# tzt101/MichiGAN

Hardware: AMD Instinct MI355X
Metric: training images/sec at 512x512 (G+D step) (higher is better)
Workload: dtype bf16; 1 GPU; SPADEB G + multiscale PatchGAN D + VGG19 + Gabor orientation losses, full G step + D step (Adam), bs=8/GPU, 512x512, BASELINE.json configs[2]; global_batch=8, batch_per_gpu=8, resolution=512, parallelism=dp1, init=reference default (xavier, 0.02), random VGG weights

## Files before the change

### michigan_amd/csrc/mg_conv_halo64.hip

```cpp
#include "mg_conv_common.h"

namespace {

constexpr int H64_PW = 18;
constexpr int H64_ROWS = H64_PW * H64_PW;
constexpr int H64_PINSTR = 44;
constexpr int H64_THREADS = 512;
constexpr int H64_PIPW = (H64_PINSTR + 7) / 8;
constexpr int H64_PBUF = H64_PINSTR * 1024;
constexpr int H64_PAR = 2 * H64_PBUF;
constexpr int H64_AUX = H64_PAR + 256;
constexpr int H64_LTMAX = 4;
constexpr int H64_LDS = H64_AUX + 8 * 4096 + H64_LTMAX * 8192;
constexpr int H64_W8 = H64_AUX + 8 * 4096;
template <int AUX> struct H64Taps { static constexpr int RT = 6, LT = 9 - RT; };
constexpr int H64_NST = 8;

struct Halo64Args {
    int units;
    int mtiles;
    int nseg;
    int tiles_per_seg;
    int bands;
    int dbg;
};

template <int ACT, int AUX>
__global__ __launch_bounds__(H64_THREADS, 2) void conv3x3_halo64_kernel(const ConvK d, const Halo64Args g)
{
    extern __shared__ __attribute__((aligned(16))) unsigned char smem[];
    const int tid = threadIdx.x, lane = tid & 63;
    const int wave = __builtin_amdgcn_readfirstlane(tid >> 6);
    const int pw = wave & 3, mw = wave >> 2;
    const int l31 = lane & 31, hi = lane >> 5;
    constexpr int H64_RT = H64Taps<AUX>::RT, H64_LT = H64Taps<AUX>::LT;

    int unit = blockIdx.x;
    if ((g.units & 7) == 0) unit = (blockIdx.x & 7) * (g.units >> 3) + (blockIdx.x >> 3);
    const int m = unit % g.mtiles;  unit /= g.mtiles;
    const int seg = unit % g.nseg;  unit /= g.nseg;
    const int band = unit % g.bands;
    const int img = unit / g.bands;
    const int m0 = m * 64 + mw * 32, y0 = band * 16, xs = seg * g.tiles_per_seg * 16;
    const int W = d.Win, H = d.Hin;

    const uint16_t* __restrict__ In = reinterpret_cast<const uint16_t*>(d.in);
    const unsigned lds0 = (unsigned)(size_t)(__attribute__((address_space(3))) unsigned char*)smem;

    bf16x8_t a[2][H64_RT][2];
    {
        const uint16_t* __restrict__ Wt = reinterpret_cast<const uint16_t*>(d.wt);
#pragma unroll
        for (int t = 0; t < H64_RT; ++t) {
            const uint16_t* row = Wt + ((size_t)t * d.CoutP + m0 + l31) * 64 + hi * 8;
#pragma unroll
            for (int c = 0; c < 2; ++c)
#pragma unroll
                for (int ks = 0; ks < 2; ++ks)
                    a[c][t][ks] = *reinterpret_cast<const bf16x8_t*>(row + c * 32 + ks * 16);
        }
    }
#pragma unroll
    for (int lt = 0; lt < H64_LT; ++lt) {
        const int row = wave * 8 + (lane >> 3), piece = (lane & 7) ^ ((row >> 1) & 7);
        glds16(reinterpret_cast<const uint16_t*>(d.wt) + ((size_t)(H64_RT + lt) * d.CoutP + m * 64 + row) * 64 + piece * 8,
               __builtin_amdgcn_readfirstlane(lds0 + H64_W8 + lt * 8192 + wave * 1024));
    }
    const int a8off = H64_W8 + (mw * 32 + l31) * 128 + ((hi ^ ((l31 >> 1) & 7)) << 4);
    if (wave == 0) {
        const void* src = (d.bias && m * 64 + lane < d.Cout_gemm) ? static_cast<const void*>(d.bias + m * 64 + lane) : static_cast<const void*>(g_mg_zeros + lane * 4);
        glds4(src, __builtin_amdgcn_readfirstlane(lds0 + H64_PAR));
    }
    const float* const par = reinterpret_cast<const float*>(smem + H64_PAR) + mw * 32;

    const unsigned char* const zsrc = g_mg_zeros + (lane & 7) * 16;
    int poff[H64_PIPW];
#pragma unroll
    for (int j = 0; j < H64_PIPW; ++j) {
        const int q = (wave + 8 * j) * 8 + (lane >> 3), s = lane & 7;
        const int pr = q / H64_PW, pc = q - pr * H64_PW;
        const int iy = y0 + pr - 1, ix = xs + pc - 1;
        const int piece = s ^ ((q >> 1) & 7);
        const bool rowok = q < H64_ROWS && (unsigned)iy < (unsigned)H;
        poff[j] = rowok ? ((int)((((long)(img * H + iy) * W + ix) * 64 + piece * 8) * 2) | (pc == 0 ? 1 : (pc == H64_PW - 1 ? 2 : 0))) : 3;
    }
    auto issue_patch = [&](int i) {
        const unsigned base = lds0 + (i & 1) * H64_PBUF;
        const int x0 = xs + i * 16;
        const bool lok = x0 > 0, rok = x0 + 16 < W;
#pragma unroll
        for (int j = 0; j < H64_PIPW; ++j) {
            if (wave + 8 * j >= H64_PINSTR) continue;
            const int cls = poff[j] & 3;
            const bool ok = cls == 0 || (cls == 1 && lok) || (cls == 2 && rok);
            const unsigned char* src = ok ? reinterpret_cast<const unsigned char*>(In) + ((long)(poff[j] & ~3) + (long)i * (16 * 64 * 2)) : zsrc;
            glds16(src, __builtin_amdgcn_readfirstlane(base + (wave + 8 * j) * 1024));
        }
    };

    int bbase[9][2];
    {
        const int py = l31 >> 4, px = (l31 - 2 * py) & 15;
#pragma unroll
        for (int t = 0; t < 9; ++t) {
            const int tp = d.tap[t];
            const int dy = (int)(short)(tp & 0xffff), dx = tp >> 16;
#pragma unroll
            for (int nt = 0; nt < 2; ++nt) {
                const int q = (pw * 4 + nt * 2 + py + 1 + dy) * H64_PW + px + 1 + dx;
                bbase[t][nt] = q * 128 + ((hi ^ ((q >> 1) & 7)) << 4);
            }
        }
    }
    unsigned ooff[2];
#pragma unroll
    for (int nt = 0; nt < 2; ++nt) {
        const int p = pw * 64 + nt * 32 + l31, py = p >> 4;
        const int y = y0 + py, x = xs + (((p & 15) - 2 * (py & 1)) & 15);
        ooff[nt] = (unsigned)(((img * d.Hout + y) * d.Wout + x) * d.Cout + m0);
    }
    uint16_t* __restrict__ Out = reinterpret_cast<uint16_t*>(d.out);
    const uint16_t* __restrict__ Aux = reinterpret_cast<const uint16_t*>(AUX == 1 ? d.resid : d.x);
    const float neg = ACT == 2 ? d.slope : 0.f;

    issue_patch(0);
    wait_vmcnt<0>();

    for (int i = 0; i < g.tiles_per_seg; ++i) {
        __builtin_amdgcn_s_barrier();
        if (i + 1 < g.tiles_per_seg && !(g.dbg & 2)) issue_patch(i + 1);
        if constexpr (AUX != 0) {
            const unsigned abase = lds0 + H64_AUX + wave * 4096;
            const uint16_t* const asrc = Aux + (hi ? ooff[1] : ooff[0]);
#pragma unroll
            for (int gq = 0; gq < 4; ++gq) glds16(asrc + gq * 8, __builtin_amdgcn_readfirstlane(abase + gq * 1024));
        }
        f32x16_t acc[2];
        const unsigned char* const Ps = smem + (i & 1) * H64_PBUF;
        if (g.dbg & 4) {
#pragma unroll
            for (int nt = 0; nt < 2; ++nt)
#pragma unroll
                for (int r = 0; r < 16; ++r) acc[nt][r] = 0.f;
        } else {
#pragma unroll
        for (int c = 0; c < 2; ++c)
#pragma unroll
            for (int t = 0; t < 9; ++t)
#pragma unroll
                for (int ks = 0; ks < 2; ++ks) {
                    bf16x8_t b[2], at;
#pragma unroll
                    for (int nt = 0; nt < 2; ++nt)
                        b[nt] = *reinterpret_cast<const bf16x8_t*>(Ps + (bbase[t][nt] ^ ((c * 4 + ks * 2) << 4)));
                    if (t < H64_RT) at = a[c][t < H64_RT ? t : 0][ks];
                    else at = *reinterpret_cast<const bf16x8_t*>(smem + (t - H64_RT) * 8192 + (a8off ^ ((c * 4 + ks * 2) << 4)));
#pragma unroll
                    for (int nt = 0; nt < 2; ++nt) {
                        if (c == 0 && t == 0 && ks == 0) {
                            const f32x16_t zero = {};
                            acc[nt] = __builtin_amdgcn_mfma_f32_32x32x16_bf16(at, b[nt], zero, 0, 0, 0);
                        } else
                            acc[nt] = __builtin_amdgcn_mfma_f32_32x32x16_bf16(at, b[nt], acc[nt], 0, 0, 0);
                    }
                }
        }
        wait_vmcnt<0>();

#pragma unroll
        for (int nt = 0; nt < 2; ++nt)
#pragma unroll
            for (int k2 = 0; k2 < 2; ++k2) {
                mg_pk2 v[4];
#pragma unroll
                for (int r2 = 0; r2 < 2; ++r2) {
                    const int rq = 2 * k2 + r2;
                    const f32x4_t bias4 = *reinterpret_cast<const f32x4_t*>(par + hi * 4 + rq * 8);
                    f32x4_t ax = {};
                    if constexpr (AUX != 0) {
                        const uint2 r = *reinterpret_cast<const uint2*>(smem + H64_AUX + wave * 4096 + rq * 1024 + (nt * 32 + l31) * 16 + hi * 8);
                        ax[0] = __uint_as_float(r.x << 16); ax[1] = __uint_as_float(r.x & 0xffff0000u);
                        ax[2] = __uint_as_float(r.y << 16); ax[3] = __uint_as_float(r.y & 0xffff0000u);
                    }
#pragma unroll
                    for (int h2 = 0; h2 < 2; ++h2) {
                        mg_pk2 tt = mg_pk(acc[nt][rq * 4 + 2 * h2], acc[nt][rq * 4 + 2 * h2 + 1]) + mg_pk(bias4[2 * h2], bias4[2 * h2 + 1]);
                        if constexpr (AUX == 1) tt += mg_pk(ax[2 * h2], ax[2 * h2 + 1]);
                        tt = mg_act2<ACT>(tt, neg);
                        if constexpr (AUX == 2) {
                            const mg_pk2 tm = tt * d.mslope;
                            tt[0] = ax[2 * h2] > 0.f ? tt[0] : tm[0];
                            tt[1] = ax[2 * h2 + 1] > 0.f ? tt[1] : tm[1];
                        }
                        v[r2 * 2 + h2] = tt;
                    }
                }
                const uint4 w = mg_pair_swap(mg_pack_bf16x2x2(v[0], v[1]), mg_pack_bf16x2x2(v[2], v[3]));
                if (!(g.dbg & 1)) *reinterpret_cast<uint4*>(Out + ooff[nt] + k2 * 16 + hi * 8) = w;
                else if (w.x == 0x12345678u) *reinterpret_cast<uint4*>(Out) = w;
            }
#pragma unroll
        for (int nt = 0; nt < 2; ++nt) ooff[nt] += 16 * d.Cout;
    }
}

template <int ACT, int AUX>
int launch64(const ConvK& k, const Halo64Args& g, hipStream_t st)
{
    auto kern = conv3x3_halo64_kernel<ACT, AUX>;
    mg_raise_lds_cap(reinterpret_cast<const void*>(kern), H64_LDS);
    hipLaunchKernelGGL(kern, dim3((unsigned)g.units), dim3(H64_THREADS), H64_LDS, st, k, g);
    MG_CHECK_LAUNCH("mg_conv_taps(halo64)");
    return MG_OK;
}

int aux_kind(const ConvK& k) { return k.resid ? (k.x ? 3 : 1) : (k.x ? 2 : 0); }
int act_kind(const ConvK& k) { return (k.act == MG_ACT_LRELU && !(k.slope >= 0.f && k.slope <= 1.f)) ? 3 : k.act; }

}

bool conv_halo64_applies(const ConvK& k, int dtype, int epilogue)
{
    if (!mg_opt(MG_OPT_CONV_HALO) || !mg_opt(MG_OPT_CONV_HALO64) || dtype != MG_BF16 || epilogue != MG_EPI_PLAIN) return false;
    if (k.Cin != 64 || k.Cout != k.Cout_gemm || (k.Cout % 64) != 0 || k.CoutP < k.Cout) return false;
    if (k.ntaps != 9 || k.isy != 1 || k.isx != 1 || k.osy != 1 || k.osx != 1 || k.ooy != 0 || k.oox != 0) return false;
    if (k.Hj != k.Hin || k.Wj != k.Win || k.Hout != k.Hin || k.Wout != k.Win) return false;
    if ((k.Hin % 16) || (k.Win % 16) || k.Hin < 32 || k.Win < 32) return false;
    if (!(k.wide & 1) || (k.wide & ~1)) return false;
    const int ak = aux_kind(k), ck = act_kind(k);
    if (!((ak == 0 && ck <= 2) || (ak <= 2 && ck == 0))) return false;
    if ((long)k.N * k.Hin * k.Win * 64 * 2 >= (1L << 31) || (long)k.N * k.Hin * k.Win * k.Cout >= (1L << 32)) return false;
    unsigned seen = 0;
    for (int t = 0; t < 9; ++t) {
        const int dy = (int)(short)(k.tap[t] & 0xffff), dx = k.tap[t] >> 16;
        if (dy < -1 || dy > 1 || dx < -1 || dx > 1) return false;
        seen |= 1u << ((dy + 1) * 3 + dx + 1);
    }
    if (seen != 0x1ffu) return false;
    if (k.Cout > 128) return false;
    return (long)k.N * (k.Hin / 16) * (k.Win / 16) * (k.Cout / 64) >= 1024;
}

int launch_conv_halo64(ConvK& k, hipStream_t st)
{
    Halo64Args g;
    g.mtiles = k.Cout / 64;
    g.bands = k.Hin / 16;
    const int tiles_x = k.Win / 16;
    const long strips = (long)k.N * g.bands * g.mtiles;
    int nseg = 1;
    while (strips * nseg < 256 && (tiles_x % (nseg * 2)) == 0 && tiles_x / (nseg * 2) >= 4) nseg *= 2;
    g.nseg = nseg;
    g.tiles_per_seg = tiles_x / nseg;
    g.units = (int)(strips * nseg);
    g.dbg = mg_opt(MG_OPT_PROBE_HALO64_DBG);
    const int ak = aux_kind(k), ck = act_kind(k);
    if (ak == 1) return launch64<0, 1>(k, g, st);
    if (ak == 2) return launch64<0, 2>(k, g, st);
    if (ck == 0) return launch64<0, 0>(k, g, st);
    if (ck == 1) return launch64<1, 0>(k, g, st);
    return launch64<2, 0>(k, g, st);
}
```

### michigan_amd/csrc/mg_conv_thin.hip

```cpp
#include "mg_conv_common.h"
#include "mg_launch.h"
#include "mg_wgrad_common.h"


namespace {

constexpr int THIN_TH = 8, THIN_TW = 32;
constexpr int THIN_HW = THIN_TW + 2, THIN_HH = THIN_TH + 2;
constexpr int THIN_HALO_BYTES = THIN_HH * THIN_HW * 16;

template <int CS>
__global__ __launch_bounds__(256, 4) void conv3x3_thin_kernel(const ConvK d, const int ntiles)
{
    constexpr int NB = 2;
    constexpr int CH = NB * 4;
    constexpr int ROW = NB * 64;
    constexpr int RPW = 2 * CS;
    extern __shared__ __attribute__((aligned(16))) unsigned char smem[];
    unsigned char* const halo = smem;
    float* const bias_s = reinterpret_cast<float*>(smem + THIN_HALO_BYTES);
    const int tid = threadIdx.x, lane = tid & 63, wave = tid >> 6, l31 = lane & 31, hi = lane >> 5;
    const int half = CS == 2 ? (wave >> 1) : 0, r0 = CS == 2 ? (wave & 1) * RPW : wave * RPW;
    const int cb = half * 64;
    unsigned char* const stage = smem + THIN_HALO_BYTES + CS * 64 * 4 + wave * (32 * ROW);

    if (tid < CS * 64) bias_s[tid] = (d.bias && tid < d.Cout_gemm) ? d.bias[tid] : 0.f;

    bf16x8_t wa[5][NB];
    int boff[5];
    const uint16_t* __restrict__ Wt = reinterpret_cast<const uint16_t*>(d.wt);
#pragma unroll
    for (int s = 0; s < 5; ++s) {
        const int t = 2 * s + hi;
        const int tc = t < 9 ? t : 8;
        const int dy = (int)(short)(d.tap[tc] & 0xffff), dx = d.tap[tc] >> 16;
        boff[s] = ((1 + dy) * THIN_HW + (1 + dx) + l31) * 16;
#pragma unroll
        for (int nb = 0; nb < NB; ++nb) {
            bf16x8_t z = {0, 0, 0, 0, 0, 0, 0, 0};
            if (t < 9) z = *reinterpret_cast<const bf16x8_t*>(Wt + ((size_t)t * d.CoutP + cb + nb * 32 + l31) * 8);
            wa[s][nb] = z;
        }
    }

    const float neg = mg_neg_slope(d.act, d.slope);
    const bool relu = d.act == MG_ACT_RELU;
    const uint16_t* __restrict__ In = reinterpret_cast<const uint16_t*>(d.in);
    unsigned char* __restrict__ Out = reinterpret_cast<unsigned char*>(d.out);
    const int tpi = d.tiles_y * d.tiles_x;

    for (int tile = blockIdx.x; tile < ntiles; tile += gridDim.x) {
        const int img = tile / tpi, tr = tile - img * tpi;
        const int y0 = (tr / d.tiles_x) * THIN_TH, x0 = (tr % d.tiles_x) * THIN_TW;
        __syncthreads();
#pragma unroll
        for (int it = 0; it < 2; ++it) {
            const int i = tid + it * 256;
            if (i < THIN_HH * THIN_HW) {
                const int hy = i / THIN_HW, hx = i - hy * THIN_HW;
                const int gy = y0 - 1 + hy, gx = x0 - 1 + hx;
                uint4 v = {0u, 0u, 0u, 0u};
                if (gy >= 0 && gy < d.Hin && gx >= 0 && gx < d.Win)
                    v = *reinterpret_cast<const uint4*>(In + ((size_t)(img * d.Hin + gy) * d.Win + gx) * 8);
                *reinterpret_cast<uint4*>(halo + i * 16) = v;
            }
        }
        __syncthreads();
#pragma unroll 1
        for (int mb = 0; mb < RPW; ++mb) {
            const int r = r0 + mb, y = y0 + r;
            if (y >= d.Hin) break;
            bf16x8_t b[5];
#pragma unroll
            for (int s = 0; s < 5; ++s) b[s] = *reinterpret_cast<const bf16x8_t*>(halo + boff[s] + r * (THIN_HW * 16));
            f32x16_t acc[NB];
#pragma unroll
            for (int nb = 0; nb < NB; ++nb)
#pragma unroll
                for (int g = 0; g < 4; ++g) {
                    const f32x4_t bq = *reinterpret_cast<const f32x4_t*>(bias_s + cb + nb * 32 + g * 8 + hi * 4);
#pragma unroll
                    for (int e = 0; e < 4; ++e) acc[nb][g * 4 + e] = bq[e];
                }
#pragma unroll
            for (int s = 0; s < 5; ++s)
#pragma unroll
                for (int nb = 0; nb < NB; ++nb)
                    acc[nb] = __builtin_amdgcn_mfma_f32_32x32x16_bf16(wa[s][nb], b[s], acc[nb], 0, 0, 0);
#pragma unroll
            for (int nb = 0; nb < NB; ++nb)
#pragma unroll
                for (int g = 0; g < 4; ++g) {
                    uint2 u;
                    u.x = f2bf2(mg_act_fast(acc[nb][g * 4 + 0], neg, relu), mg_act_fast(acc[nb][g * 4 + 1], neg, relu));
                    u.y = f2bf2(mg_act_fast(acc[nb][g * 4 + 2], neg, relu), mg_act_fast(acc[nb][g * 4 + 3], neg, relu));
                    const int c = nb * 4 + g;
                    *reinterpret_cast<uint2*>(stage + l31 * ROW + ((c ^ ((l31 >> 1) & (CH - 1))) << 4) + hi * 8) = u;
                }
            __builtin_amdgcn_fence(__ATOMIC_RELEASE, "wavefront");
            __builtin_amdgcn_wave_barrier();
            const size_t orow = (size_t)(img * d.Hout + y) * d.Wout + x0;
#pragma unroll
            for (int it = 0; it < CH / 2; ++it) {
                const int q = it * 64 + lane;
                const int p = q / CH, c = q % CH;
                const uint4 v = *reinterpret_cast<const uint4*>(stage + p * ROW + ((c ^ ((p >> 1) & (CH - 1))) << 4));
                const int co = cb + c * 8;
                if (co < d.Cout)
                    *reinterpret_cast<uint4*>(Out + ((orow + p) * d.Cout + co) * 2) = v;
            }
            __builtin_amdgcn_fence(__ATOMIC_ACQUIRE, "wavefront");
            __builtin_amdgcn_wave_barrier();
        }
    }
}

template <int CS>
int launch_thin(ConvK& k, hipStream_t st)
{
    k.tiles_y = (k.Hin + THIN_TH - 1) / THIN_TH;
    k.tiles_x = k.Win / THIN_TW;
    const long ntiles = (long)k.N * k.tiles_y * k.tiles_x;
    if (ntiles <= 0 || ntiles > 0x7fffffffL) return mg_fail(MG_ERR_ARG, "mg_conv_taps(thin): bad grid %ld", ntiles);
    const int lds = THIN_HALO_BYTES + CS * 64 * 4 + 4 * 32 * 128;
    const long grid = ntiles < 1024 ? ntiles : 1024;
    hipLaunchKernelGGL(conv3x3_thin_kernel<CS>, dim3((unsigned)grid), dim3(256), lds, st, k, (int)ntiles);
    MG_CHECK_LAUNCH("mg_conv_taps(thin)");
    return MG_OK;
}


template <int CS, int S>
__global__ __launch_bounds__(256, 2) void conv_thin_taps_kernel(const ConvK d, const int ntiles, const int HH, const int HW,
                                                                const int dy0, const int dx0, const int nsteps)
{
    constexpr int NB = 2, CH = NB * 4, ROW = NB * 64, RPW = 2 * CS, RB = 2, WROWS = CS * 64;
    extern __shared__ __attribute__((aligned(16))) unsigned char smem[];
    const int tid = threadIdx.x, lane = tid & 63, wave = tid >> 6, l31 = lane & 31, hi = lane >> 5;
    const int half = CS == 2 ? (wave >> 1) : 0, r0 = CS == 2 ? (wave & 1) * RPW : wave * RPW;
    const int cb = half * 64;
    unsigned char* const wl = smem;
    unsigned char* const halo = wl + nsteps * 2 * WROWS * 16;
    int* const tofs = reinterpret_cast<int*>(halo + HH * HW * 16);
    float* const bias_s = reinterpret_cast<float*>(tofs + MG_MAX_TAPS);
    unsigned char* const stage = reinterpret_cast<unsigned char*>(bias_s + WROWS) + wave * (32 * ROW);

    if (tid < WROWS) bias_s[tid] = (d.bias && tid < d.Cout_gemm) ? d.bias[tid] : 0.f;
    if (tid < MG_MAX_TAPS) {
        int v = 0;
#pragma unroll
        for (int t = 0; t < MG_MAX_TAPS; ++t) v = (tid == t) ? d.tap[t] : v;
        tofs[tid] = v;
    }
    {
        const uint16_t* __restrict__ Wt = reinterpret_cast<const uint16_t*>(d.wt);
        for (int i = tid; i < nsteps * 2 * WROWS; i += 256) {
            const int t = i / WROWS, row = i % WROWS;
            uint4 v = {0u, 0u, 0u, 0u};
            if (t < d.ntaps) v = *reinterpret_cast<const uint4*>(Wt + ((size_t)t * d.CoutP + row) * 8);
            *reinterpret_cast<uint4*>(wl + i * 16) = v;
        }
    }
    const float neg = mg_neg_slope(d.act, d.slope);
    const bool relu = d.act == MG_ACT_RELU;
    const uint16_t* __restrict__ In = reinterpret_cast<const uint16_t*>(d.in);
    unsigned char* __restrict__ Out = reinterpret_cast<unsigned char*>(d.out);
    const int tpi = d.tiles_y * d.tiles_x;
    const unsigned char* const wa = wl + (hi * WROWS + cb + l31) * 16;

    constexpr int HPT = 6;
    uint4 hv[HPT];
    const int npix = HH * HW;
    auto fetch = [&](int tile) {
        const int img = tile / tpi, tr = tile - img * tpi;
        const int y0 = (tr / d.tiles_x) * THIN_TH, x0 = (tr % d.tiles_x) * THIN_TW;
#pragma unroll
        for (int q = 0; q < HPT; ++q) {
            const int i = tid + q * 256;
            const int hy = i / HW, hx = i - hy * HW;
            const int gy = y0 * S + dy0 + hy, gx = x0 * S + dx0 + hx;
            uint4 v = {0u, 0u, 0u, 0u};
            if (i < npix && gy >= 0 && gy < d.Hin && gx >= 0 && gx < d.Win)
                v = *reinterpret_cast<const uint4*>(In + ((size_t)(img * d.Hin + gy) * d.Win + gx) * 8);
            hv[q] = v;
        }
    };
    if ((int)blockIdx.x < ntiles) fetch(blockIdx.x);
    for (int tile = blockIdx.x; tile < ntiles; tile += gridDim.x) {
        const int img = tile / tpi, tr = tile - img * tpi;
        const int y0 = (tr / d.tiles_x) * THIN_TH, x0 = (tr % d.tiles_x) * THIN_TW;
        __syncthreads();
#pragma unroll
        for (int q = 0; q < HPT; ++q) {
            const int i = tid + q * 256;
            if (i < npix) *reinterpret_cast<uint4*>(halo + i * 16) = hv[q];
        }
        __syncthreads();
        if (tile + (int)gridDim.x < ntiles) fetch(tile + gridDim.x);
#pragma unroll 1
        for (int rg = 0; rg < RPW; rg += RB) {
        if (y0 + r0 + rg >= d.Hj) break;
        const unsigned char* const bb = halo + (((r0 + rg) * S) * HW + l31 * S) * 16;
        f32x16_t acc[RB][NB];
#pragma unroll
        for (int mb = 0; mb < RB; ++mb)
#pragma unroll
            for (int nb = 0; nb < NB; ++nb)
#pragma unroll
                for (int g = 0; g < 4; ++g) {
                    const f32x4_t bq = *reinterpret_cast<const f32x4_t*>(bias_s + cb + nb * 32 + g * 8 + hi * 4);
#pragma unroll
                    for (int e = 0; e < 4; ++e) acc[mb][nb][g * 4 + e] = bq[e];
                }
#pragma unroll 5
        for (int s = 0; s < nsteps; ++s) {
            const int o = tofs[2 * s + hi];
            const bf16x8_t a0 = *reinterpret_cast<const bf16x8_t*>(wa + s * (2 * WROWS * 16));
            const bf16x8_t a1 = *reinterpret_cast<const bf16x8_t*>(wa + s * (2 * WROWS * 16) + 32 * 16);
#pragma unroll
            for (int mb = 0; mb < RB; ++mb) {
                const bf16x8_t b = *reinterpret_cast<const bf16x8_t*>(bb + o + mb * (S * HW * 16));
                acc[mb][0] = __builtin_amdgcn_mfma_f32_32x32x16_bf16(a0, b, acc[mb][0], 0, 0, 0);
                acc[mb][1] = __builtin_amdgcn_mfma_f32_32x32x16_bf16(a1, b, acc[mb][1], 0, 0, 0);
            }
        }
#pragma unroll
        for (int mb = 0; mb < RB; ++mb) {
            const int y = y0 + r0 + rg + mb;
            if (y >= d.Hj) break;
#pragma unroll
            for (int nb = 0; nb < NB; ++nb)
#pragma unroll
                for (int g = 0; g < 4; ++g) {
                    uint2 u;
                    u.x = f2bf2(mg_act_fast(acc[mb][nb][g * 4 + 0], neg, relu), mg_act_fast(acc[mb][nb][g * 4 + 1], neg, relu));
                    u.y = f2bf2(mg_act_fast(acc[mb][nb][g * 4 + 2], neg, relu), mg_act_fast(acc[mb][nb][g * 4 + 3], neg, relu));
                    const int c = nb * 4 + g;
                    *reinterpret_cast<uint2*>(stage + l31 * ROW + ((c ^ ((l31 >> 1) & (CH - 1))) << 4) + hi * 8) = u;
                }
            __builtin_amdgcn_fence(__ATOMIC_RELEASE, "wavefront");
            __builtin_amdgcn_wave_barrier();
            const size_t orow = (size_t)(img * d.Hout + y) * d.Wout + x0;
            const int pmax = d.Wout - x0;
#pragma unroll
            for (int it = 0; it < CH / 2; ++it) {
                const int q = it * 64 + lane;
                const int p = q / CH, c = q % CH;
                const uint4 v = *reinterpret_cast<const uint4*>(stage + p * ROW + ((c ^ ((p >> 1) & (CH - 1))) << 4));
                const int co = cb + c * 8;
                if (co < d.Cout && p < pmax)
                    *reinterpret_cast<uint4*>(Out + ((orow + p) * d.Cout + co) * 2) = v;
            }
            __builtin_amdgcn_fence(__ATOMIC_ACQUIRE, "wavefront");
            __builtin_amdgcn_wave_barrier();
        }
        }
    }
}

struct ThinTapsGeom { int S, dy0, dx0, KH, KW, HH, HW, nsteps, CS, lds; long ntiles; };

bool thin_taps_geom(const ConvK& k, ThinTapsGeom& g)
{
    if (k.isy != k.isx || (k.isy != 1 && k.isy != 2) || k.ntaps > 50) return false;
    int dy0 = 127, dx0 = 127, dy1 = -128, dx1 = -128;
    for (int t = 0; t < k.ntaps; ++t) {
        const int dy = (int)(short)(k.tap[t] & 0xffff), dx = k.tap[t] >> 16;
        dy0 = dy < dy0 ? dy : dy0; dy1 = dy > dy1 ? dy : dy1; dx0 = dx < dx0 ? dx : dx0; dx1 = dx > dx1 ? dx : dx1;
    }
    g.S = k.isy; g.dy0 = dy0; g.dx0 = dx0; g.KH = dy1 - dy0 + 1; g.KW = dx1 - dx0 + 1;
    if (g.KH > 7 || g.KW > 7) return false;
    g.HH = (THIN_TH - 1) * g.S + g.KH; g.HW = (THIN_TW - 1) * g.S + g.KW;
    g.nsteps = (k.ntaps + 1) / 2;
    g.CS = k.Cout_gemm <= 64 ? 1 : 2;
    g.lds = g.nsteps * 2 * g.CS * 64 * 16 + g.HH * g.HW * 16 + MG_MAX_TAPS * 4 + g.CS * 64 * 4 + 4 * 32 * 128;
    g.ntiles = (long)k.N * ((k.Hj + THIN_TH - 1) / THIN_TH) * ((k.Wj + THIN_TW - 1) / THIN_TW);
    return g.lds <= 80 * 1024 && g.ntiles >= 64 && g.ntiles <= 0x7fffffffL;
}

template <int CS, int S>
int launch_thin_taps(ConvK& k, const ThinTapsGeom& g, hipStream_t st)
{
    k.tiles_y = (k.Hj + THIN_TH - 1) / THIN_TH;
    k.tiles_x = (k.Wj + THIN_TW - 1) / THIN_TW;
    int ofs[MG_MAX_TAPS];
    for (int t = 0; t < MG_MAX_TAPS; ++t) {
        const int tc = t < k.ntaps ? t : 0;
        const int dy = (int)(short)(k.tap[tc] & 0xffff), dx = k.tap[tc] >> 16;
        ofs[t] = ((dy - g.dy0) * g.HW + (dx - g.dx0)) * 16;
    }
    for (int t = 0; t < MG_MAX_TAPS; ++t) k.tap[t] = ofs[t];
    auto kern = conv_thin_taps_kernel<CS, S>;
    mg_raise_lds_cap(reinterpret_cast<const void*>(kern), 80 * 1024);
    const long grid = g.ntiles < 512 ? g.ntiles : 512;
    hipLaunchKernelGGL(kern, dim3((unsigned)grid), dim3(256), g.lds, st, k, (int)g.ntiles, g.HH, g.HW, g.dy0, g.dx0, g.nsteps);
    MG_CHECK_LAUNCH("mg_conv_taps(thin, tap list)");
    return MG_OK;
}

typedef __attribute__((ext_vector_type(4))) short thin_s16x4_t;
typedef __attribute__((address_space(3))) thin_s16x4_t* thin_lds_s16x4_p;
constexpr int WTH = 4;
constexpr int WHALO_BYTES = (WTH + 2) * THIN_HW * 16;

template <int MB>
__global__ __launch_bounds__(256, MB == 4 ? 3 : 4) void wgrad3x3_thin_kernel(const Wg3K d, const int ntiles, const int tiles_y, const int tiles_x)
{
    constexpr int RBA = MB * 64, PPA = RBA / 16;
    constexpr int KG = 4 / MB;
    constexpr int APT = WTH * 32 * PPA / 256;
    extern __shared__ __attribute__((aligned(16))) unsigned char smem[];
    unsigned char* const halo = smem;
    unsigned char* const dyt = smem + WHALO_BYTES;
    const int tid = threadIdx.x, lane = tid & 63, wave = tid >> 6, l31 = lane & 31, hi = lane >> 5;
    const int mblk = wave % MB, kg = wave / MB;
    auto swz = [](int row) { return RBA == 256 ? (row & 3) : ((row >> 1) & 1); };

    const int i16 = lane & 15, g2 = lane >> 4;
    const int rsub = (g2 >> 1) * 8 + (i16 >> 2);
    const int csub = ((g2 & 1) * 16 + (i16 & 3) * 4) * 2;
    int boff[3];
#pragma unroll
    for (int nb = 0; nb < 3; ++nb) {
        const int n = nb * 32 + (g2 & 1) * 16 + (i16 & 3) * 4;
        const int tap = (n >> 3) < 9 ? (n >> 3) : 8;
        boff[nb] = ((tap / 3) * THIN_HW + rsub + tap % 3) * 16 + ((n >> 2) & 1) * 8;
    }

    f32x16_t acc[3];
#pragma unroll
    for (int nb = 0; nb < 3; ++nb)
#pragma unroll
        for (int r = 0; r < 16; ++r) acc[nb][r] = 0.f;
    float bsum = 0.f;

    const uint16_t* __restrict__ X = reinterpret_cast<const uint16_t*>(d.x);
    const uint16_t* __restrict__ DY = reinterpret_cast<const uint16_t*>(d.dy);
    const int tpi = tiles_y * tiles_x;

    uint4 hv = {0u, 0u, 0u, 0u};
    uint4 av[APT];
    auto fetch = [&](int tile) {
        const int img = tile / tpi, tr = tile - img * tpi;
        const int y0 = (tr / tiles_x) * WTH, x0 = (tr % tiles_x) * THIN_TW;
        if (tid < (WTH + 2) * THIN_HW) {
            const int hy = tid / THIN_HW, hx = tid - hy * THIN_HW;
            const int gy = y0 - 1 + hy, gx = x0 - 1 + hx;
            uint4 v = {0u, 0u, 0u, 0u};
            if (gy >= 0 && gy < d.H && gx >= 0 && gx < d.W)
                v = *reinterpret_cast<const uint4*>(X + ((size_t)(img * d.H + gy) * d.W + gx) * 8);
            hv = v;
        }
#pragma unroll
        for (int j = 0; j < APT; ++j) {
            const int g = j * 256 + tid, prow = g / PPA, slot = g % PPA;
            const int y = y0 + (prow >> 5), x = x0 + (prow & 31);
            uint4 v = {0u, 0u, 0u, 0u};
            if (y < d.H) v = *reinterpret_cast<const uint4*>(DY + ((size_t)(img * d.H + y) * d.W + x) * d.Cg + slot * 8);
            av[j] = v;
        }
    };
    if ((int)blockIdx.x < ntiles) fetch(blockIdx.x);
    for (int tile = blockIdx.x; tile < ntiles; tile += gridDim.x) {
        __syncthreads();
        if (tid < (WTH + 2) * THIN_HW) *reinterpret_cast<uint4*>(halo + tid * 16) = hv;
#pragma unroll
        for (int j = 0; j < APT; ++j) {
            const int g = j * 256 + tid, prow = g / PPA, slot = g % PPA;
            *reinterpret_cast<uint4*>(dyt + prow * RBA + ((slot ^ (swz(prow) << 2)) << 4)) = av[j];
        }
        __syncthreads();
        if (tile + (int)gridDim.x < ntiles) fetch(tile + gridDim.x);
#pragma unroll
        for (int kk = 0; kk < WTH * 2 / KG; ++kk) {
            const int kstep = kk * KG + kg, r = kstep >> 1, ks = kstep & 1;
            const int pr = r * 32 + ks * 16 + rsub;
            const unsigned char* pa = dyt + pr * RBA + ((mblk * 64 + csub) ^ (swz(pr) << 6));
            const thin_s16x4_t a0 = __builtin_amdgcn_ds_read_tr16_b64_v4i16((thin_lds_s16x4_p)(pa));
            const thin_s16x4_t a1 = __builtin_amdgcn_ds_read_tr16_b64_v4i16((thin_lds_s16x4_p)(pa + 4 * RBA));
            const bf16x8_t a = __builtin_bit_cast(bf16x8_t, __builtin_shufflevector(a0, a1, 0, 1, 2, 3, 4, 5, 6, 7));
            {
                typedef __attribute__((ext_vector_type(4))) unsigned u32x4_t;
                const u32x4_t w = __builtin_bit_cast(u32x4_t, a);
#pragma unroll
                for (int j = 0; j < 4; ++j) bsum += __uint_as_float(w[j] << 16) + __uint_as_float(w[j] & 0xffff0000u);
            }
            const unsigned char* pb = halo + (r * THIN_HW + ks * 16) * 16;
#pragma unroll
            for (int nb = 0; nb < 3; ++nb) {
                const thin_s16x4_t b0 = __builtin_amdgcn_ds_read_tr16_b64_v4i16((thin_lds_s16x4_p)(pb + boff[nb]));
                const thin_s16x4_t b1 = __builtin_amdgcn_ds_read_tr16_b64_v4i16((thin_lds_s16x4_p)(pb + boff[nb] + 64));
                const bf16x8_t b = __builtin_bit_cast(bf16x8_t, __builtin_shufflevector(b0, b1, 0, 1, 2, 3, 4, 5, 6, 7));
                acc[nb] = __builtin_amdgcn_mfma_f32_32x32x16_bf16(a, b, acc[nb], 0, 0, 0);
            }
        }
    }

    const int split = blockIdx.x * KG + kg;
    if (d.dbias) {
        const float t = bsum + __shfl_xor(bsum, 32);
        if (hi == 0) wg_accum(d.dbias, d.det_stride, split, (size_t)(mblk * 32 + l31), t);
    }
#pragma unroll
    for (int nb = 0; nb < 3; ++nb) {
        const int n = nb * 32 + l31, tap = n >> 3, ci = n & 7;
        if (tap < 9) {
#pragma unroll
            for (int r = 0; r < 16; ++r) {
                const int co = mblk * 32 + (r & 3) + 8 * (r >> 2) + 4 * hi;
                wg_accum(d.dw, d.det_stride, split, (size_t)(tap * d.Cg + co) * 8 + ci, acc[nb][r]);
            }
        }
    }
}


template <int NBW, int S>
__global__ __launch_bounds__(256, 2) void wgrad_thin_taps_kernel(const WgT d, const int ntiles, const int tiles_y, const int tiles_x)
{
    constexpr int RBA = 128, PPA = 8;
    constexpr int APT = WTH * 32 * PPA / 256;
    extern __shared__ __attribute__((aligned(16))) unsigned char smem[];
    const int hbytes = d.HH * d.HW * 16;
    unsigned char* const halo = smem;
    unsigned char* const dyt = smem + hbytes;
    int* const tofs = reinterpret_cast<int*>(dyt + WTH * 32 * RBA);
    const int tid = threadIdx.x, lane = tid & 63, wave = tid >> 6, l31 = lane & 31, hi = lane >> 5;
    const int mblk = wave & 1, ng = wave >> 1;
    auto swz = [](int row) { return (row >> 1) & 1; };

    if (tid < MG_MAX_TAPS) {
        int v = 0;
#pragma unroll
        for (int t = 0; t < MG_MAX_TAPS; ++t) v = (tid == t) ? d.tap[t] : v;
        tofs[tid] = v;
    }
    __syncthreads();
    const int i16 = lane & 15, g2 = lane >> 4;
    const int rsub = (g2 >> 1) * 8 + (i16 >> 2);
    const int csub = ((g2 & 1) * 16 + (i16 & 3) * 4) * 2;
    int boff[NBW];
#pragma unroll
    for (int nb = 0; nb < NBW; ++nb) {
        const int n = (ng * NBW + nb) * 32 + (g2 & 1) * 16 + (i16 & 3) * 4;
        const int tap = (n >> 3) < d.ntaps ? (n >> 3) : 0;
        boff[nb] = (tofs[tap] + rsub * S) * 16 + ((n >> 2) & 1) * 8;
    }

    f32x16_t acc[NBW];
#pragma unroll
    for (int nb = 0; nb < NBW; ++nb)
#pragma unroll
        for (int r = 0; r < 16; ++r) acc[nb][r] = 0.f;
    float bsum = 0.f;

    const uint16_t* __restrict__ X = reinterpret_cast<const uint16_t*>(d.x);
    const uint16_t* __restrict__ DY = reinterpret_cast<const uint16_t*>(d.dy);
    const int tpi = tiles_y * tiles_x;

    constexpr int HPT = 3;
    uint4 hv[HPT];
    uint4 av[APT];
    const int npix = d.HH * d.HW;
    auto fetch = [&](int tile) {
        const int img = tile / tpi, tr = tile - img * tpi;
        const int y0 = (tr / tiles_x) * WTH, x0 = (tr % tiles_x) * THIN_TW;
#pragma unroll
        for (int q = 0; q < HPT; ++q) {
            const int i = tid + q * 256;
            const int hy = i / d.HW, hx = i - hy * d.HW;
            const int gy = y0 * S + d.dy0 + hy, gx = x0 * S + d.dx0 + hx;
            uint4 v = {0u, 0u, 0u, 0u};
            if (i < npix && gy >= 0 && gy < d.Hin && gx >= 0 && gx < d.Win)
                v = *reinterpret_cast<const uint4*>(X + ((size_t)(img * d.Hin + gy) * d.Win + gx) * 8);
            hv[q] = v;
        }
#pragma unroll
        for (int j = 0; j < APT; ++j) {
            const int g = j * 256 + tid, prow = g / PPA, slot = g % PPA;
            const int y = y0 + (prow >> 5), x = x0 + (prow & 31);
            uint4 v = {0u, 0u, 0u, 0u};
            if (y < d.Hj && x < d.Wj) v = *reinterpret_cast<const uint4*>(DY + ((size_t)(img * d.Hj + y) * d.Wj + x) * 64 + slot * 8);
            av[j] = v;
        }
    };
    if ((int)blockIdx.x < ntiles) fetch(blockIdx.x);
    for (int tile = blockIdx.x; tile < ntiles; tile += gridDim.x) {
        __syncthreads();
#pragma unroll
        for (int q = 0; q < HPT; ++q) {
            const int i = tid + q * 256;
            if (i < npix) *reinterpret_cast<uint4*>(halo + i * 16) = hv[q];
        }
#pragma unroll
        for (int j = 0; j < APT; ++j) {
            const int g = j * 256 + tid, prow = g / PPA, slot = g % PPA;
            *reinterpret_cast<uint4*>(dyt + prow * RBA + ((slot ^ (swz(prow) << 2)) << 4)) = av[j];
        }
        __syncthreads();
        if (tile + (int)gridDim.x < ntiles) fetch(tile + gridDim.x);
#pragma unroll 2
        for (int kstep = 0; kstep < WTH * 2; ++kstep) {
            const int r = kstep >> 1, ks = kstep & 1;
            const int pr = r * 32 + ks * 16 + rsub;
            const unsigned char* pa = dyt + pr * RBA + ((mblk * 64 + csub) ^ (swz(pr) << 6));
            const thin_s16x4_t a0 = __builtin_amdgcn_ds_read_tr16_b64_v4i16((thin_lds_s16x4_p)(pa));
            const thin_s16x4_t a1 = __builtin_amdgcn_ds_read_tr16_b64_v4i16((thin_lds_s16x4_p)(pa + 4 * RBA));
            const bf16x8_t a = __builtin_bit_cast(bf16x8_t, __builtin_shufflevector(a0, a1, 0, 1, 2, 3, 4, 5, 6, 7));
            if (ng == 0) {
                typedef __attribute__((ext_vector_type(4))) unsigned u32x4_t;
                const u32x4_t w = __builtin_bit_cast(u32x4_t, a);
#pragma unroll
                for (int j = 0; j < 4; ++j) bsum += __uint_as_float(w[j] << 16) + __uint_as_float(w[j] & 0xffff0000u);
            }
            const unsigned char* pb = halo + ((r * S) * d.HW + ks * 16 * S) * 16;
#pragma unroll
            for (int nb = 0; nb < NBW; ++nb) {
                const thin_s16x4_t b0 = __builtin_amdgcn_ds_read_tr16_b64_v4i16((thin_lds_s16x4_p)(pb + boff[nb]));
                const thin_s16x4_t b1 = __builtin_amdgcn_ds_read_tr16_b64_v4i16((thin_lds_s16x4_p)(pb + boff[nb] + 64 * S));
                const bf16x8_t b = __builtin_bit_cast(bf16x8_t, __builtin_shufflevector(b0, b1, 0, 1, 2, 3, 4, 5, 6, 7));
                acc[nb] = __builtin_amdgcn_mfma_f32_32x32x16_bf16(a, b, acc[nb], 0, 0, 0);
            }
        }
    }

    float* const slab = d.ws + (size_t)blockIdx.x * d.slab;
    if (d.has_bias && ng == 0) {
        const float t = bsum + __shfl_xor(bsum, 32);
        if (hi == 0) slab[(size_t)d.ntaps * 64 * 8 + mblk * 32 + l31] = t;
    }
#pragma unroll
    for (int nb = 0; nb < NBW; ++nb) {
        const int n = (ng * NBW + nb) * 32 + l31, tap = n >> 3, ci = n & 7;
        if (tap < d.ntaps) {
#pragma unroll
            for (int r = 0; r < 16; ++r) {
                const int co = mblk * 32 + (r & 3) + 8 * (r >> 2) + 4 * hi;
                slab[(size_t)(tap * 64 + co) * 8 + ci] = acc[nb][r];
            }
        }
    }
}

template <int NBW, int S>
int launch_wthin_taps(const WgT& k, int grid, long ntiles, int tiles_y, int tiles_x, hipStream_t st)
{
    const int lds = k.HH * k.HW * 16 + WTH * 32 * 128 + MG_MAX_TAPS * 4;
    hipLaunchKernelGGL((wgrad_thin_taps_kernel<NBW, S>), dim3((unsigned)grid), dim3(256), lds, st, k, (int)ntiles, tiles_y, tiles_x);
    MG_CHECK_LAUNCH("mg_conv_wgrad(thin, tap list)");
    return MG_OK;
}

template <int MB>
int launch_wthin(Wg3K& k, hipStream_t st, int* nsplit, bool dry)
{
    const int tiles_y = (k.H + WTH - 1) / WTH, tiles_x = k.W / THIN_TW;
    const long ntiles = (long)k.N * tiles_y * tiles_x;
    if (ntiles <= 0 || ntiles > 0x7fffffffL) return mg_fail(MG_ERR_ARG, "mg_conv_wgrad(thin): bad grid %ld", ntiles);
    long grid = (ntiles + 3) / 4;
    if (grid > 512) grid = 512;
    if (nsplit) *nsplit = (int)grid * (4 / MB);
    if (dry) return MG_OK;
    const int lds = WHALO_BYTES + WTH * 32 * MB * 64;
    hipLaunchKernelGGL(wgrad3x3_thin_kernel<MB>, dim3((unsigned)grid), dim3(256), lds, st, k, (int)ntiles, tiles_y, tiles_x);
    MG_CHECK_LAUNCH("mg_conv_wgrad(thin)");
    return MG_OK;
}

}

bool conv_thin_applies(const ConvK& k, int dtype, int epilogue)
{
    if (!mg_opt(MG_OPT_CONV_THIN) || dtype != MG_BF16 || epilogue != MG_EPI_PLAIN) return false;
    if (k.Cin != 8 || k.ntaps != 9 || k.isy != 1 || k.isx != 1 || k.osy != 1 || k.osx != 1 || k.ooy != 0 || k.oox != 0) return false;
    if (k.Hj != k.Hin || k.Wj != k.Win || k.Hout != k.Hin || k.Wout != k.Win) return false;
    if (k.resid || k.x || k.act == MG_ACT_TANH) return false;
    if ((k.Win % THIN_TW) || (k.Cout & 7) || k.Cout_gemm > 128 || k.Cout_gemm < 32) return false;
    unsigned seen = 0;
    for (int t = 0; t < 9; ++t) {
        const int dy = (int)(short)(k.tap[t] & 0xffff), dx = k.tap[t] >> 16;
        if (dy < -1 || dy > 1 || dx < -1 || dx > 1) return false;
        seen |= 1u << ((dy + 1) * 3 + dx + 1);
    }
    if (seen != 0x1ffu) return false;
    return (long)k.N * ((k.Hin + THIN_TH - 1) / THIN_TH) * (k.Win / THIN_TW) >= 64;
}

bool conv_thin_taps_applies(const ConvK& k, int dtype, int epilogue)
{
    if (mg_opt(MG_OPT_CONV_THIN) < 2 || dtype != MG_BF16 || epilogue != MG_EPI_PLAIN) return false;
    if (k.Cin != 8 || k.osy != 1 || k.osx != 1 || k.ooy != 0 || k.oox != 0 || k.Hout != k.Hj || k.Wout != k.Wj) return false;
    if (k.resid || k.x || k.act == MG_ACT_TANH || (k.Cout & 7) || k.Cout_gemm > 128 || k.Cout_gemm < 32) return false;
    ThinTapsGeom g;
    return thin_taps_geom(k, g);
}

int launch_conv_thin_taps(ConvK& k, hipStream_t st)
{
    ThinTapsGeom g;
    if (!thin_taps_geom(k, g)) return mg_fail(MG_ERR_UNSUPPORTED, "mg_conv_taps(thin, tap list): geometry");
    if (g.CS == 1) return g.S == 1 ? launch_thin_taps<1, 1>(k, g, st) : launch_thin_taps<1, 2>(k, g, st);
    return g.S == 1 ? launch_thin_taps<2, 1>(k, g, st) : launch_thin_taps<2, 2>(k, g, st);
}

int launch_conv_thin(ConvK& k, hipStream_t st)
{
    if (k.Cout_gemm <= 64) return launch_thin<1>(k, st);
    return launch_thin<2>(k, st);
}

bool wgrad_thin_applies(const Wg3K& k)
{
    return mg_opt(MG_OPT_CONV_THIN) && k.Cin == 8 && (k.Cg == 64 || k.Cg == 128) && (k.W % THIN_TW) == 0 &&
           (long)k.N * ((k.H + WTH - 1) / WTH) * (k.W / THIN_TW) >= 64;
}

int launch_wgrad_thin(Wg3K& k, hipStream_t st, int* nsplit, bool dry)
{
    return k.Cg == 64 ? launch_wthin<2>(k, st, nsplit, dry) : launch_wthin<4>(k, st, nsplit, dry);
}

static bool wgrad_thin_taps_geom(const mg_wgrad_desc* d, WgT& k, long& ntiles, int& tiles_y, int& tiles_x, int& nblocks)
{
    if (mg_opt(MG_OPT_CONV_THIN) < 2 || d->dtype != MG_BF16 || d->Cin != 8 || d->Cg != 64 || d->isy != d->isx || (d->isy != 1 && d->isy != 2)) return false;
    if (d->ntaps > 52) return false;
    int dy0 = 127, dx0 = 127, dy1 = -128, dx1 = -128;
    for (int t = 0; t < d->ntaps; ++t) {
        const int dy = d->tap_dy[t], dx = d->tap_dx[t];
        dy0 = dy < dy0 ? dy : dy0; dy1 = dy > dy1 ? dy : dy1; dx0 = dx < dx0 ? dx : dx0; dx1 = dx > dx1 ? dx : dx1;
    }
    const int KH = dy1 - dy0 + 1, KW = dx1 - dx0 + 1, S = d->isy;
    if (KH > 7 || KW > 7) return false;
    k.x = d->x; k.dy = d->dy; k.ws = nullptr; k.N = d->N; k.Hin = d->Hin; k.Win = d->Win; k.Hj = d->Hj; k.Wj = d->Wj; k.ntaps = d->ntaps;
    k.dy0 = dy0; k.dx0 = dx0; k.HH = (WTH - 1) * S + KH; k.HW = (THIN_TW - 1) * S + KW;
    k.slab = (long)d->ntaps * 64 * 8 + (d->dbias ? 64 : 0); k.has_bias = d->dbias ? 1 : 0;
    for (int t = 0; t < MG_MAX_TAPS; ++t) {
        const int tc = t < d->ntaps ? t : 0;
        k.tap[t] = (d->tap_dy[tc] - dy0) * k.HW + (d->tap_dx[tc] - dx0);
    }
    tiles_y = (d->Hj + WTH - 1) / WTH; tiles_x = (d->Wj + THIN_TW - 1) / THIN_TW;
    ntiles = (long)d->N * tiles_y * tiles_x;
    nblocks = (d->ntaps * 8 + 31) / 32;
    return ntiles >= 64 && ntiles <= 0x7fffffffL;
}

bool wgrad_thin_taps_applies(const mg_wgrad_desc* d)
{
    WgT k; long ntiles; int ty, tx, nb;
    return wgrad_thin_taps_geom(d, k, ntiles, ty, tx, nb);
}

int launch_wgrad_thin_taps(const mg_wgrad_desc* d, hipStream_t st, float* dw, float* dbias, long det_stride, int* nsplit, bool dry)
{
    WgT k; long ntiles; int tiles_y, tiles_x, nblocks;
    if (!wgrad_thin_taps_geom(d, k, ntiles, tiles_y, tiles_x, nblocks)) return mg_fail(MG_ERR_UNSUPPORTED, "mg_conv_wgrad(thin, tap list): geometry");
    long grid = (ntiles + 7) / 8;
    if (grid > 512) grid = 512;
    if (nsplit) *nsplit = (int)grid;
    if (dry) return MG_OK;
    const long ndw = (long)d->ntaps * 64 * 8;
    if (det_stride) {
        if (det_stride != k.slab) return mg_fail(MG_ERR_ARG, "mg_conv_wgrad(thin, tap list): slab stride %ld, expected %ld", det_stride, k.slab);
        k.ws = dw;
    } else {
        k.ws = mg_stream_scratch(st, (size_t)grid * k.slab * sizeof(float));
        if (k.ws == nullptr) return mg_fail(MG_ERR_LAUNCH, "mg_conv_wgrad(thin, tap list): scratch allocation failed");
    }
    const int S = d->isy;
    int rc;
    if (nblocks <= 4) rc = S == 1 ? launch_wthin_taps<2, 1>(k, (int)grid, ntiles, tiles_y, tiles_x, st) : launch_wthin_taps<2, 2>(k, (int)grid, ntiles, tiles_y, tiles_x, st);
    else if (nblocks <= 8) rc = S == 1 ? launch_wthin_taps<4, 1>(k, (int)grid, ntiles, tiles_y, tiles_x, st) : launch_wthin_taps<4, 2>(k, (int)grid, ntiles, tiles_y, tiles_x, st);
    else rc = S == 1 ? launch_wthin_taps<7, 1>(k, (int)grid, ntiles, tiles_y, tiles_x, st) : launch_wthin_taps<7, 2>(k, (int)grid, ntiles, tiles_y, tiles_x, st);
    if (rc != MG_OK || det_stride) return rc;
    return launch_wgrad_det_finish(k.ws, (int)grid, k.slab, dw, ndw, dbias, d->dbias ? 64 : 0, st);
}
```

Measured before the change: 130.7 images/s.

## Stage thin wgrad partials in LDS for coalesced flush and shrink split grid

```diff
diff --git a/michigan_amd/csrc/mg_conv_halo64.hip b/michigan_amd/csrc/mg_conv_halo64.hip
--- a/michigan_amd/csrc/mg_conv_halo64.hip
+++ b/michigan_amd/csrc/mg_conv_halo64.hip
@@ -30,6 +30,7 @@
 {
     extern __shared__ __attribute__((aligned(16))) unsigned char smem[];
     const int tid = threadIdx.x, lane = tid & 63;
+    const int dbg = MG_PROBES ? g.dbg : 0;
     const int wave = __builtin_amdgcn_readfirstlane(tid >> 6);
     const int pw = wave & 3, mw = wave >> 2;
     const int l31 = lane & 31, hi = lane >> 5;
@@ -128,7 +129,7 @@
 
     for (int i = 0; i < g.tiles_per_seg; ++i) {
         __builtin_amdgcn_s_barrier();
-        if (i + 1 < g.tiles_per_seg && !(g.dbg & 2)) issue_patch(i + 1);
+        if (i + 1 < g.tiles_per_seg && !(dbg & 2)) issue_patch(i + 1);
         if constexpr (AUX != 0) {
             const unsigned abase = lds0 + H64_AUX + wave * 4096;
             const uint16_t* const asrc = Aux + (hi ? ooff[1] : ooff[0]);
@@ -137,7 +138,7 @@
         }
         f32x16_t acc[2];
         const unsigned char* const Ps = smem + (i & 1) * H64_PBUF;
-        if (g.dbg & 4) {
+        if (dbg & 4) {
 #pragma unroll
             for (int nt = 0; nt < 2; ++nt)
 #pragma unroll
@@ -196,7 +197,7 @@
                     }
                 }
                 const uint4 w = mg_pair_swap(mg_pack_bf16x2x2(v[0], v[1]), mg_pack_bf16x2x2(v[2], v[3]));
-                if (!(g.dbg & 1)) *reinterpret_cast<uint4*>(Out + ooff[nt] + k2 * 16 + hi * 8) = w;
+                if (!(dbg & 1)) *reinterpret_cast<uint4*>(Out + ooff[nt] + k2 * 16 + hi * 8) = w;
                 else if (w.x == 0x12345678u) *reinterpret_cast<uint4*>(Out) = w;
             }
 #pragma unroll
@@ -253,7 +254,7 @@
     g.nseg = nseg;
     g.tiles_per_seg = tiles_x / nseg;
     g.units = (int)(strips * nseg);
-    g.dbg = mg_opt(MG_OPT_PROBE_HALO64_DBG);
+    g.dbg = MG_PROBES ? mg_opt(MG_OPT_PROBE_HALO64_DBG) : 0;
     const int ak = aux_kind(k), ck = act_kind(k);
     if (ak == 1) return launch64<0, 1>(k, g, st);
     if (ak == 2) return launch64<0, 2>(k, g, st);
diff --git a/michigan_amd/csrc/mg_conv_thin.hip b/michigan_amd/csrc/mg_conv_thin.hip
--- a/michigan_amd/csrc/mg_conv_thin.hip
+++ b/michigan_amd/csrc/mg_conv_thin.hip
@@ -302,6 +302,13 @@
 typedef __attribute__((address_space(3))) thin_s16x4_t* thin_lds_s16x4_p;
 constexpr int WTH = 4;
 constexpr int WHALO_BYTES = (WTH + 2) * THIN_HW * 16;
+constexpr int WFLUSH_FLOATS = 9 * 32 * 8;
+#ifndef MG_WTHIN_MIN_TILES
+#define MG_WTHIN_MIN_TILES 0
+#endif
+#ifndef MG_WTHIN_MAX_GRID
+#define MG_WTHIN_MAX_GRID 0
+#endif
 
 template <int MB>
 __global__ __launch_bounds__(256, MB == 4 ? 3 : 4) void wgrad3x3_thin_kernel(const Wg3K d, const int ntiles, const int tiles_y, const int tiles_x)
@@ -401,17 +408,20 @@
         const float t = bsum + __shfl_xor(bsum, 32);
         if (hi == 0) wg_accum(d.dbias, d.det_stride, split, (size_t)(mblk * 32 + l31), t);
     }
+    __syncthreads();
+    float* const wl = reinterpret_cast<float*>(smem) + wave * WFLUSH_FLOATS;
 #pragma unroll
     for (int nb = 0; nb < 3; ++nb) {
         const int n = nb * 32 + l31, tap = n >> 3, ci = n & 7;
         if (tap < 9) {
 #pragma unroll
-            for (int r = 0; r < 16; ++r) {
-                const int co = mblk * 32 + (r & 3) + 8 * (r >> 2) + 4 * hi;
-                wg_accum(d.dw, d.det_stride, split, (size_t)(tap * d.Cg + co) * 8 + ci, acc[nb][r]);
-            }
-        }
-    }
+            for (int r = 0; r < 16; ++r) wl[(tap * 32 + (r & 3) + 8 * (r >> 2) + 4 * hi) * 8 + ci] = acc[nb][r];
+        }
+    }
+    __syncthreads();
+#pragma unroll 4
+    for (int i = lane; i < WFLUSH_FLOATS; i += 64)
+        wg_accum(d.dw, d.det_stride, split, (size_t)(i >> 8) * d.Cg * 8 + mblk * 256 + (i & 255), wl[i]);
 }
 
 
@@ -557,11 +567,14 @@
     const int tiles_y = (k.H + WTH - 1) / WTH, tiles_x = k.W / THIN_TW;
     const long ntiles = (long)k.N * tiles_y * tiles_x;
     if (ntiles <= 0 || ntiles > 0x7fffffffL) return mg_fail(MG_ERR_ARG, "mg_conv_wgrad(thin): bad grid %ld", ntiles);
-    long grid = (ntiles + 3) / 4;
-    if (grid > 512) grid = 512;
+    const long mint = MG_WTHIN_MIN_TILES ? MG_WTHIN_MIN_TILES : (ntiles >= 1024 ? 8 : 4);
+    long grid = (ntiles + mint - 1) / mint;
+    const long cap = MG_WTHIN_MAX_GRID ? MG_WTHIN_MAX_GRID : (ntiles >= 16 * 512 ? 512 : 256);
+    if (grid > cap) grid = cap;
     if (nsplit) *nsplit = (int)grid * (4 / MB);
     if (dry) return MG_OK;
-    const int lds = WHALO_BYTES + WTH * 32 * MB * 64;
+    const int tile_lds = WHALO_BYTES + WTH * 32 * MB * 64, flush_lds = 4 * WFLUSH_FLOATS * 4;
+    const int lds = tile_lds > flush_lds ? tile_lds : flush_lds;
     hipLaunchKernelGGL(wgrad3x3_thin_kernel<MB>, dim3((unsigned)grid), dim3(256), lds, st, k, (int)ntiles, tiles_y, tiles_x);
     MG_CHECK_LAUNCH("mg_conv_wgrad(thin)");
     return MG_OK;
```

After: 131.0 images/s (median of 2 runs). About the same (+0.2%).
